# pangenome/gfasort

Hardware: AMD Instinct MI355X
Metric: SGD term-updates/sec, -p Y, 1M-node synthetic GFA (higher is better)
Workload: dtype f64

## Files before the change

gfasort_amd/csrc/host/graph.cpp:

```cpp
#include "graph.hpp"

#include <algorithm>
#include <atomic>
#include <cerrno>
#include <chrono>
#include <cstdlib>
#include <cstdio>
#include <cstring>
#include <exception>
#include <functional>
#include <stdexcept>
#include <thread>

#include <sched.h>

namespace gfasort {

namespace {
std::atomic<size_t> g_io_threads{0};

void parallel_for_impl(size_t n, const std::function<void(size_t)> &fn) {
    size_t nt = std::min(io_threads(), n);
    if (nt <= 1) { for (size_t i = 0; i < n; ++i) fn(i); return; }
    std::atomic<size_t> next{0};
// ... 79 lines not shown
        }
        add_edge(list[k].from, list[k].to);
    }
}

bool BidirectedGraph::has_edge(Handle from, Handle to) const {
    return edges.count(BiEdge{from, to}) || edges.count(BiEdge{to.flip(), from.flip()});
}

size_t BidirectedGraph::node_count() const {
    size_t n = 0;
    for (const auto &x : nodes) n += x.has_value();
    return n;
}

std::vector<size_t> BidirectedGraph::seeding_order() const {
    if (!node_order.empty()) return node_order;
    std::vector<size_t> ids;
    for (size_t id = 0; id < nodes.size(); ++id) if (nodes[id].has_value()) ids.push_back(id);
    return ids;
}

FlatGraph BidirectedGraph::flatten() const {
    FlatGraph f;
    std::vector<uint32_t> idx_of(nodes.size(), GFS_NO_NODE);
    for (size_t id : seeding_order()) {
        if (id < nodes.size() && nodes[id].has_value()) {
            if (idx_of[id] != GFS_NO_NODE) continue;
            idx_of[id] = (uint32_t)f.node_len.size();
            f.node_len.push_back((uint32_t)nodes[id]->sequence.size());
            f.node_ids.push_back(id);
        }
    }
    f.path_first_step.push_back(0);
    for (const auto &p : paths)
        f.path_first_step.push_back(f.path_first_step.back() + p.steps.size());
    f.step_node.resize(f.path_first_step.back());
    f.step_is_rev.resize(f.path_first_step.back());
    const auto chunks = step_chunks(paths, (size_t)1 << 18);
    parallel_for(chunks.size(), [&](size_t c) {
        const StepChunk &ck = chunks[c];
        const Handle *st = paths[ck.path].steps.data();
        uint32_t *sn = f.step_node.data() + f.path_first_step[ck.path];
        uint8_t *sr = f.step_is_rev.data() + f.path_first_step[ck.path];
        for (size_t k = ck.begin; k < ck.end; ++k) {
            size_t id = st[k].node_id();
            sn[k] = id < idx_of.size() ? idx_of[id] : GFS_NO_NODE;
            sr[k] = st[k].is_reverse() ? 1 : 0;
        }
    });
    return f;
}

void BidirectedGraph::apply_ordering(const std::vector<Handle> &ordering) {
    if (ordering.empty()) return;
    size_t max_old = nodes.size();
    for (Handle h : ordering) max_old = std::max(max_old, h.node_id() + 1);
    std::vector<size_t> old_to_new(max_old, 0);
    for (size_t k = 0; k < ordering.size(); ++k) old_to_new[ordering[k].node_id()] = k + 1;
    auto lookup = [&](size_t id) -> size_t { return id < old_to_new.size() ? old_to_new[id] : 0; };
    size_t max_new = 0;
    for (size_t v : old_to_new) max_new = std::max(max_new, v);
    std::vector<std::optional<BiNode>> new_nodes(max_new + 1);
    {
        const size_t BLOCK = (size_t)1 << 16;
        parallel_for((nodes.size() + BLOCK - 1) / BLOCK, [&](size_t b) {
            for (size_t id = b * BLOCK; id < std::min(nodes.size(), (b + 1) * BLOCK); ++id) {
                size_t nid = lookup(id);
                if (nid && nodes[id].has_value()) {
                    BiNode n = std::move(*nodes[id]);
                    n.id = nid;
                    n.rank = (uint64_t)(nid - 1);
                    new_nodes[nid] = std::move(n);
                }
            }
        });
    }
    nodes = std::move(new_nodes);
    std::vector<BiEdge> relabelled(edges.begin(), edges.end());
    {
        std::vector<uint8_t> keep(relabelled.size(), 0);
        const size_t BLOCK = (size_t)1 << 16;
        parallel_for((relabelled.size() + BLOCK - 1) / BLOCK, [&](size_t b) {
            for (size_t k = b * BLOCK; k < std::min(relabelled.size(), (b + 1) * BLOCK); ++k) {
                const BiEdge e = relabelled[k];
                size_t f = lookup(e.from.node_id()), t = lookup(e.to.node_id());
                if (f && t) { relabelled[k] = BiEdge{Handle::make(f, e.from.is_reverse()), Handle::make(t, e.to.is_reverse())}; keep[k] = 1; }
            }
        });
        size_t n = 0;
        for (size_t k = 0; k < relabelled.size(); ++k) if (keep[k]) relabelled[n++] = relabelled[k];
        relabelled.resize(n);
    }
    EdgeSet new_edges;
    new_edges.reserve(relabelled.size());
    for (size_t k = 0; k < relabelled.size(); ++k) {
        if (k + 16 < relabelled.size()) new_edges.prefetch(relabelled[k + 16]);
        new_edges.insert(relabelled[k]);
    }
    edges = std::move(new_edges);
    const auto chunks = step_chunks(paths, (size_t)1 << 18);
    parallel_for(chunks.size(), [&](size_t c) {
        const StepChunk &ck = chunks[c];
        Handle *st = paths[ck.path].steps.data();
        for (size_t k = ck.begin; k < ck.end; ++k) {
            size_t nid = lookup(st[k].node_id());
            if (nid) st[k] = Handle::make(nid, st[k].is_reverse());
        }
    });
}

namespace {
inline void put_uint(std::string &b, uint64_t v) {
    char tmp[24]; int n = 24;
    do { tmp[--n] = (char)('0' + v % 10); v /= 10; } while (v);
    b.append(tmp + n, (size_t)(24 - n));
}
}

namespace {
void write_blocks(std::ostream &out, size_t n, size_t block, const std::function<void(size_t, size_t, std::string &)> &fmt) {
    const size_t nblocks = (n + block - 1) / block;
    const size_t window = std::max<size_t>(io_threads() * 4, 1);
    std::vector<std::string> piece(std::min(window, std::max<size_t>(nblocks, 1)));
    for (size_t base = 0; base < nblocks; base += window) {
        const size_t cnt = std::min(window, nblocks - base);
        parallel_for(cnt, [&](size_t i) {
            piece[i].clear();
            fmt((base + i) * block, std::min(n, (base + i + 1) * block), piece[i]);
        });
        for (size_t i = 0; i < cnt; ++i) out.write(piece[i].data(), (std::streamsize)piece[i].size());
    }
}
}

void BidirectedGraph::write_gfa(std::ostream &out) const {
    const bool timing = std::getenv("GFS_TIMING") != nullptr;
    auto t_prev = std::chrono::steady_clock::now();
    auto lap = [&](const char *what) {
        if (!timing) return;
        auto t = std::chrono::steady_clock::now();
        std::fprintf(stderr, "[write_gfa] %-10s %8.2f ms\n", what, std::chrono::duration<double, std::milli>(t - t_prev).count());
        t_prev = t;
    };
    std::string b;
    b.reserve(9u << 20);
    auto flush = [&](bool force) { if (force || b.size() > (8u << 20)) { out.write(b.data(), (std::streamsize)b.size()); b.clear(); } };
    b += "H\tVN:Z:1.0\n";
    flush(true);
    write_blocks(out, nodes.size(), (size_t)1 << 16, [&](size_t lo, size_t hi, std::string &o) {
        for (size_t id = lo; id < hi; ++id)
            if (nodes[id].has_value()) {
                o += "S\t"; put_uint(o, id); o.push_back('\t'); o += nodes[id]->sequence; o.push_back('\n');
            }
    });
    lap("S");
    std::vector<BiEdge> es(edges.begin(), edges.end());
    lap("L copy");
    {
        auto less = [](const BiEdge &a, const BiEdge &c) { return a.from.v != c.from.v ? a.from.v < c.from.v : a.to.v < c.to.v; };
        size_t runs = 1;
        while (runs * 2 <= io_threads() && es.size() / (runs * 2) >= 65536) runs *= 2;
        auto bound = [&](size_t r, size_t of) { return es.size() * r / of; };
        parallel_for(runs, [&](size_t r) { std::sort(es.begin() + (std::ptrdiff_t)bound(r, runs), es.begin() + (std::ptrdiff_t)bound(r + 1, runs), less); });
        for (size_t width = 1; width < runs; width *= 2)
            parallel_for(runs / (2 * width), [&](size_t m) {
                const size_t lo = bound(2 * width * m, runs), mid = bound(2 * width * m + width, runs), hi = bound(2 * width * (m + 1), runs);
                std::inplace_merge(es.begin() + (std::ptrdiff_t)lo, es.begin() + (std::ptrdiff_t)mid, es.begin() + (std::ptrdiff_t)hi, less);
            });
    }
    lap("L sort");
    write_blocks(out, es.size(), (size_t)1 << 16, [&](size_t lo, size_t hi, std::string &o) {
        o.reserve((hi - lo) * 28);
        for (size_t k = lo; k < hi; ++k) {
            const BiEdge &e = es[k];
            o += "L\t"; put_uint(o, e.from.node_id()); o.push_back('\t'); o.push_back(e.from.orientation_char());
            o.push_back('\t'); put_uint(o, e.to.node_id()); o.push_back('\t'); o.push_back(e.to.orientation_char());
            o += "\t0M\n";
        }
    });
    lap("L");
    const auto chunks = step_chunks(paths, (size_t)1 << 17);
    const size_t window = std::max<size_t>(io_threads() * 4, 1);
    std::vector<std::string> piece(std::min(window, chunks.size()));
    size_t next_path = 0;
    auto header = [&](size_t p) { b += "P\t"; b += paths[p].name; b.push_back('\t'); };
    auto close_paths_before = [&](size_t p, bool started) {
        if (started) b += "\t*\n";
        for (; next_path < p; ++next_path) { header(next_path); b += "\t*\n"; }
    };
    bool started = false;
    for (size_t base = 0; base < chunks.size(); base += window) {
        const size_t n = std::min(window, chunks.size() - base);
        parallel_for(n, [&](size_t i) {
            const StepChunk &ck = chunks[base + i];
            const Handle *st = paths[ck.path].steps.data();
            std::string &o = piece[i];
            o.clear();
            o.reserve((ck.end - ck.begin) * 10);
            for (size_t k = ck.begin; k < ck.end; ++k) {
                if (k) o.push_back(',');
                put_uint(o, st[k].node_id()); o.push_back(st[k].orientation_char());
            }
        });
        for (size_t i = 0; i < n; ++i) {
            const StepChunk &ck = chunks[base + i];
            if (ck.begin == 0) {
                close_paths_before(ck.path, started);
                header(ck.path); next_path = ck.path + 1; started = true;
            }
            flush(true);
            out.write(piece[i].data(), (std::streamsize)piece[i].size());
        }
    }
    close_paths_before(paths.size(), started);
    flush(true);
    lap("P");
}

namespace {
struct Line { const char *b, *e; };
inline bool field(const Line &ln, int k, const char *&fb, const char *&fe) {
    const char *p = ln.b;
    for (int i = 0; i < k; ++i) {
        const char *t = (const char *)memchr(p, '\t', (size_t)(ln.e - p));
        if (!t) return false;
        p = t + 1;
    }
    const char *t = (const char *)memchr(p, '\t', (size_t)(ln.e - p));
    fb = p; fe = t ? t : ln.e;
    return true;
}
inline int count_fields(const Line &ln) {
    int n = 1;
    for (const char *p = ln.b; (p = (const char *)memchr(p, '\t', (size_t)(ln.e - p))); ++p) ++n;
    return n;
}
size_t parse_usize(const char *b, const char *e, const char *what) {
    if (b < e && *b == '+') ++b;
    if (b >= e) throw std::runtime_error(std::string("Failed to parse ") + what + ": cannot parse integer from empty string");
    uint64_t v = 0;
    for (; b < e; ++b) {
        if (*b < '0' || *b > '9') throw std::runtime_error(std::string("Failed to parse ") + what + ": invalid digit found in string");
        const uint64_t d = (uint64_t)(*b - '0');
        if (v > 1844674407370955161ull || (v == 1844674407370955161ull && d > 5))
            throw std::runtime_error(std::string("Failed to parse ") + what + ": number too large to fit in target type");
        v = v * 10 + d;
    }
    return (size_t)v;
}
}

BidirectedGraph parse_gfa(const std::string &content) {
    BidirectedGraph g;
    const bool timing = std::getenv("GFS_TIMING") != nullptr;
// ... 168 lines not shown
```

gfasort_amd/csrc/host/graph.hpp:

```cpp
#pragma once
#include <cstdint>
#include <functional>
#include <optional>
#include <ostream>
#include <string>
#include <iterator>
#include <vector>

#include "../../../include/gfasort_hip.h"

namespace gfasort {

struct Handle {
    uint64_t v = 0;
    static Handle make(size_t node_id, bool is_reverse) { return Handle{((uint64_t)node_id << 1) | (is_reverse ? 1u : 0u)}; }
    static Handle forward(size_t node_id) { return make(node_id, false); }
    static Handle reverse(size_t node_id) { return make(node_id, true); }
    static Handle from_u64(uint64_t x) { return Handle{x}; }
    size_t node_id() const { return (size_t)(v >> 1); }
    bool is_reverse() const { return (v & 1) == 1; }
    char orientation_char() const { return is_reverse() ? '-' : '+'; }
    Handle flip() const { return Handle{v ^ 1}; }
    uint64_t as_u64() const { return v; }
    bool operator==(const Handle &o) const { return v == o.v; }
// ... 34 lines not shown
        const BiEdge *operator->() const { return &s_->slots_[i_]; }
        const_iterator &operator++() { ++i_; skip(); return *this; }
        bool operator!=(const const_iterator &o) const { return i_ != o.i_; }
        bool operator==(const const_iterator &o) const { return i_ == o.i_; }
        using iterator_category = std::forward_iterator_tag;
        using value_type = BiEdge; using difference_type = std::ptrdiff_t;
        using pointer = const BiEdge *; using reference = const BiEdge &;
    private:
        void skip() { while (i_ < s_->used_.size() && !s_->used_[i_]) ++i_; }
        const EdgeSet *s_; size_t i_;
    };
    size_t size() const { return n_; }
    bool empty() const { return n_ == 0; }
    void clear() { slots_.clear(); used_.clear(); n_ = 0; }
    void reserve(size_t n) { if (n * 10 > slots_.size() * 7) rehash(n); }
    size_t count(const BiEdge &e) const {
        if (slots_.empty()) return 0;
        const size_t mask = slots_.size() - 1;
        for (size_t i = BiEdgeHash()(e) & mask;; i = (i + 1) & mask) {
            if (!used_[i]) return 0;
            if (slots_[i] == e) return 1;
        }
    }
    bool insert(const BiEdge &e) {
        if ((n_ + 1) * 10 > slots_.size() * 7) rehash(n_ + 1);
        const size_t mask = slots_.size() - 1;
        for (size_t i = BiEdgeHash()(e) & mask;; i = (i + 1) & mask) {
            if (!used_[i]) { slots_[i] = e; used_[i] = 1; ++n_; return true; }
            if (slots_[i] == e) return false;
        }
    }
    void prefetch(const BiEdge &e) const {
        if (slots_.empty()) return;
        const size_t i = BiEdgeHash()(e) & (slots_.size() - 1);
        __builtin_prefetch(&slots_[i]); __builtin_prefetch(&used_[i]);
    }
    const_iterator begin() const { return const_iterator(this, 0); }
    const_iterator end() const { return const_iterator(this, used_.size()); }
private:
    void rehash(size_t want) {
        size_t cap = 16;
        while (cap * 7 < want * 10) cap <<= 1;
        if (cap < slots_.size()) cap = slots_.size();
        std::vector<BiEdge> old_s(cap); std::vector<uint8_t> old_u(cap, 0);
        old_s.swap(slots_); old_u.swap(used_);
        n_ = 0;
        for (size_t i = 0; i < old_u.size(); ++i) if (old_u[i]) insert(old_s[i]);
    }
    std::vector<BiEdge> slots_;
    std::vector<uint8_t> used_;
    size_t n_ = 0;
};

struct FlatGraph {
    std::vector<uint32_t> node_len;
    std::vector<uint32_t> step_node;
    std::vector<uint8_t> step_is_rev;
    std::vector<uint64_t> path_first_step;
    std::vector<size_t> node_ids;
    gfs_graph_view view() const {
        gfs_graph_view v;
        v.n_nodes = node_len.size(); v.n_steps = step_node.size(); v.n_paths = path_first_step.size() - 1;
        v.node_len = node_len.data(); v.step_node = step_node.data();
        v.step_is_rev = step_is_rev.data(); v.path_first_step = path_first_step.data();
        return v;
    }
};

struct BidirectedGraph {
    std::vector<std::optional<BiNode>> nodes;
    EdgeSet edges;
    std::vector<BiPath> paths;
    std::vector<size_t> node_order;

    void add_node(size_t id, std::string sequence);
    void add_edge(Handle from, Handle to);
    void add_edges(const std::vector<BiEdge> &list);
    bool has_edge(Handle from, Handle to) const;
    size_t node_count() const;
    void apply_ordering(const std::vector<Handle> &ordering);
    void write_gfa(std::ostream &out) const;
    std::vector<size_t> seeding_order() const;
    FlatGraph flatten() const;
};

void set_io_threads(size_t n);
size_t io_threads();
void parallel_for(size_t n, const std::function<void(size_t)> &fn);

std::string read_file(const std::string &path);

BidirectedGraph parse_gfa(const std::string &content);

}
```

gfasort_amd/csrc/host/main.cpp:

```cpp
#include <chrono>
#include <cstdlib>
#include <cstring>
#include <fstream>
#include <iostream>
#include <sstream>
#include <string>
#include <thread>

#include "sgd.hpp"

using namespace gfasort;

struct Args {
    std::string input, output, pipeline = "sYgs", layout_out;
    size_t iter_max = 100, threads = 1, dimensions = 2, layout_iter = 30;
    unsigned verbose = 1;
    uint64_t streams = 0; uint32_t flags = 0;
    unsigned bundle = 0;
    bool reference_sampler = false, phased = false;
};

static void usage() {
    std::cerr <<
        "Usage: gfasort_hip -i <in.gfa> -o <out.gfa> [-p PIPELINE] [--iter-max N] [-t N] [-v N]\n"
// ... 20 lines not shown
        std::string f = argv[i];
        const char *v;
        if (f == "-i" || f == "--input") { if (!(v = need(i))) return false; a.input = v; }
        else if (f == "-o" || f == "--output") { if (!(v = need(i))) return false; a.output = v; }
        else if (f == "-p" || f == "--pipeline") { if (!(v = need(i))) return false; a.pipeline = v; }
        else if (f == "--iter-max") { if (!(v = need(i))) return false; a.iter_max = std::stoull(v); }
        else if (f == "-t" || f == "--threads") { if (!(v = need(i))) return false; a.threads = std::stoull(v); }
        else if (f == "-v" || f == "--verbose") { if (!(v = need(i))) return false; a.verbose = (unsigned)std::stoul(v); }
        else if (f == "--dimensions") { if (!(v = need(i))) return false; a.dimensions = std::stoull(v); }
        else if (f == "--layout-out") { if (!(v = need(i))) return false; a.layout_out = v; }
        else if (f == "--layout-iter") { if (!(v = need(i))) return false; a.layout_iter = std::stoull(v); }
        else if (f == "--io-threads") { if (!(v = need(i))) return false; set_io_threads(std::stoull(v)); }
        else if (f == "--streams") { if (!(v = need(i))) return false; a.streams = std::stoull(v); }
        else if (f == "--bundle") { if (!(v = need(i))) return false; a.bundle = std::string(v) == "auto" ? 0u : (unsigned)std::stoul(v); }
        else if (f == "--reference-sampler") { a.bundle = 1; a.reference_sampler = true; }
        else if (f == "--phased-sampler") { a.phased = true; }
        else if (f == "--hip-flags") { if (!(v = need(i))) return false; a.flags = (uint32_t)std::stoul(v); }
        else if (f == "-h" || f == "--help") { usage(); exit(0); }
        else { std::cerr << "error: unexpected argument '" << f << "'\n"; return false; }
    }
    if (a.phased && (a.reference_sampler || (a.bundle != 0 && a.bundle != 64))) {
        std::cerr << "error: --phased-sampler switches between the reference sampler and bundles of 64: not with --reference-sampler or --bundle "
                  << a.bundle << "\n";
        return false;
    }
    if (a.input.empty() || a.output.empty()) { std::cerr << "error: -i and -o are required\n"; return false; }
    return true;
}

static int validate_pipeline(const std::string &p) {
    for (char c : p) {
        switch (c) {
            case 'Y': case 'L': break;
            case 'g': case 's': case 'S': case 'u':
                std::cerr << "Error: pipeline step '" << c << "' is part of the reference but not of this build "
                             "(only Y = SGD and L = layout run on the HIP engine)\n";
                return 1;
            default:
                std::cerr << "Error: Unknown pipeline character '" << c
                          << "'. Valid: Y (SGD), g (groom), s (topo-sort), S (priority-topo-sort), u (unchop), L (layout)\n";
                return 1;
        }
    }
    if (p.empty()) { std::cerr << "Error: Pipeline cannot be empty\n"; return 1; }
    return 0;
}

int main(int argc, char **argv) {
    Args args;
    if (!parse_args(argc, argv, args)) { usage(); return 2; }
    if (validate_pipeline(args.pipeline)) return 1;
    auto t_start = std::chrono::steady_clock::now();
    auto since = [&](std::chrono::steady_clock::time_point t0) { return std::chrono::duration<double>(std::chrono::steady_clock::now() - t0).count(); };
    double t_read = 0, t_parse = 0, t_steps = 0, t_write = 0;
    std::thread warm([] { (void)gfs_warmup(0); });
    struct Joiner { std::thread &t; ~Joiner() { if (t.joinable()) t.join(); } } joiner{warm};
    if (args.verbose >= 1) std::cerr << "[gfasort] reading " << args.input << "\n";
    std::string content;
    try { content = read_file(args.input); }
    catch (const std::exception &e) { std::cerr << "Error reading file: " << e.what() << "\n"; return 1; }
    t_read = since(t_start);
    auto t_p0 = std::chrono::steady_clock::now();
    BidirectedGraph graph;
    try { graph = parse_gfa(content); }
    catch (const std::exception &e) { std::cerr << "Error parsing GFA: " << e.what() << "\n"; return 1; }
    t_parse = since(t_p0);
    if (args.verbose >= 1)
        std::cerr << "[gfasort] loaded " << graph.node_count() << " nodes, " << graph.edges.size() << " edges, "
                  << graph.paths.size() << " paths\n";
    if (args.verbose >= 2) std::cerr << "[gfasort] pipeline: " << args.pipeline << "\n";

    YgsParams ygs = YgsParams::from_graph(graph, (uint8_t)args.verbose, args.threads);
    PathSGDParams sgd_params = ygs.path_sgd;
    sgd_params.iter_max = args.iter_max;
    LayoutSGDParams layout_params = LayoutSGDParams::from_graph(graph, args.dimensions, args.threads);
    layout_params.iter_max = args.layout_iter;
    layout_params.progress = args.verbose >= 2;
    HipOptions opt; opt.cfg.n_streams = args.streams; opt.cfg.flags = args.flags | GFS_F_BUNDLE(args.bundle);

    bool have_layout = false;
    Layout layout;
    auto t_s0 = std::chrono::steady_clock::now();
    try {
        size_t step = 0;
        for (char c : args.pipeline) {
            ++step;
            if (args.verbose >= 1)
                std::cerr << "[gfasort] [" << step << "/" << args.pipeline.size() << "] "
                          << (c == 'Y' ? std::string("SGD") : std::to_string(args.dimensions) + "D layout") << "\n";
            gfs_stats st{};
            if (c == 'Y') {
                HipOptions opt_y = opt;
                if (args.phased) opt_y.cfg.flags |= GFS_F_PHASED;
                sgd_sort_only(graph, sgd_params, (uint8_t)args.verbose, opt_y, &st);
                if (args.phased && args.verbose >= 2) {
                    uint64_t kb = 0, ke = sgd_params.iter_max + 1;
                    if (st.bundle == 64) { gfs_sgd_params cp = sgd_params.to_c(); gfs_phase_window(&cp, &kb, &ke); }
                    std::cerr << "[gfasort_hip] phased sampler: reference streams in iterations [" << kb << ", " << ke << ") of 0.."
                              << sgd_params.iter_max << "\n";
                }
            } else {
                layout = path_linear_sgd_layout(graph, layout_params, opt, &st);
                have_layout = true;
                if (args.verbose >= 1) {
                    double stress = calculate_layout_stress(graph, layout, 10000);
                    char buf[64]; snprintf(buf, sizeof buf, "%.6f", stress);
                    std::cerr << "[gfasort] layout stress: " << buf << "\n";
                }
            }
            if (args.verbose >= 1 && st.iterations)
                std::cerr << "[gfasort_hip] " << st.term_updates << " term updates in " << st.iterations << " iterations on "
                          << st.n_streams << " streams (bundle " << st.bundle << "); kernels " << st.kernel_ms << " ms ("
                          << (st.kernel_ms > 0 ? (double)st.term_updates / st.kernel_ms / 1e6 : 0.0) << " G updates/s), call "
                          << st.total_ms << " ms\n";
        }
    } catch (const std::exception &e) {
        std::cerr << "Error: " << e.what() << "\n";
        return 1;
    }
    t_steps = since(t_s0);
    if (warm.joinable()) warm.join();
    auto t_w0 = std::chrono::steady_clock::now();
    if (have_layout) {
        if (!args.layout_out.empty()) {
            if (args.verbose >= 1) std::cerr << "[gfasort] writing layout to " << args.layout_out << "\n";
            std::ofstream f(args.layout_out, std::ios::binary);
            if (!f) { std::cerr << "Error creating layout file: " << std::strerror(errno) << "\n"; return 1; }
            layout.write_tsv(f);
        } else if (args.verbose >= 1) {
            std::cerr << "[gfasort] warning: layout computed but --layout-out not specified\n";
        }
    }
    if (args.verbose >= 1) std::cerr << "[gfasort] writing " << args.output << "\n";
    {
        std::ofstream f(args.output, std::ios::binary);
        if (!f) { std::cerr << "Error writing output file: " << std::strerror(errno) << "\n"; return 1; }
        graph.write_gfa(f);
    }
    t_write = since(t_w0);
    if (args.verbose >= 1) {
        double s = std::chrono::duration<double>(std::chrono::steady_clock::now() - t_start).count();
        std::cerr << "[gfasort] done (" << s << " s wall: read " << t_read << ", parse " << t_parse << ", pipeline "
                  << t_steps << ", write " << t_write << ")\n";
    }
    std::cerr.flush(); std::cout.flush();
    std::_Exit(0);
}
```

gfasort_amd/csrc/host/selftest.cpp:

```cpp
#include <cmath>
#include <fstream>
#include <iostream>
#include <sstream>

#include "sgd.hpp"

using namespace gfasort;
#define REQUIRE(c) do { if (!(c)) { std::cerr << "FAIL " << __FILE__ << ":" << __LINE__ << " " #c "\n"; return 1; } } while (0)

static std::string slurp(const std::string &p) { std::ifstream f(p, std::ios::binary); std::ostringstream s; s << f.rdbuf(); return s.str(); }

int main(int argc, char **argv) {
    std::string data = argc > 1 ? argv[1] : "tests/data";
    {
        Handle h1 = Handle::forward(42);
        REQUIRE(h1.node_id() == 42 && !h1.is_reverse() && h1.orientation_char() == '+');
        Handle h2 = Handle::reverse(42);
        REQUIRE(h2.node_id() == 42 && h2.is_reverse() && h2.orientation_char() == '-');
        REQUIRE(h2.as_u64() == 85 && Handle::from_u64(85) == h2);
        Handle h3 = Handle::forward(10).flip();
        REQUIRE(h3.node_id() == 10 && h3.is_reverse() && h3.flip() == Handle::forward(10));
        REQUIRE(Handle::reverse(7).to_string() == "7-");
        std::cout << "ok handle\n";
    }
// ... 23 lines not shown
        REQUIRE((g.node_order == std::vector<size_t>{1, 2, 3}));
        g.apply_ordering({});
        REQUIRE(g.node_count() == 3);
        std::cout << "ok graph\n";
    }
    {
        Layout l(2, 10);
        REQUIRE(l.coords.size() == 40);
        Layout m(2, 5);
        m.set(2, 0, 0, 100); m.set(2, 0, 1, 200); m.set(2, 1, 0, 150); m.set(2, 1, 1, 250);
        REQUIRE(m.get(2, 0, 0) == 100 && m.get(2, 0, 1) == 200 && m.get(2, 1, 0) == 150 && m.get(2, 1, 1) == 250);
        Layout d(2, 2); d.set(1, 0, 0, 3); d.set(1, 0, 1, 4);
        REQUIRE(std::fabs(d.distance(0, 0, 1, 0) - 5.0) < 1e-10);
        Layout v = Layout::from_vectors({{1, 2, 3, 4}, {10, 20, 30, 40}});
        REQUIRE(v.num_nodes == 2 && v.dimensions == 2 && v.get(0, 0, 0) == 1 && v.get(0, 0, 1) == 10 && v.get(0, 1, 0) == 2
                && v.get(0, 1, 1) == 20 && v.get(1, 0, 0) == 3 && v.get(1, 0, 1) == 30);
        Layout t(2, 1); t.set(0, 0, 0, 1.5); t.set(0, 0, 1, 10.0); t.set(0, 1, 0, 0.1 + 0.2); t.set(0, 1, 1, 1e21);
        std::ostringstream out; t.write_tsv(out);
        REQUIRE(out.str() == "idx\tx+\ty+\tx-\ty-\n0\t1.5\t10\t0.30000000000000004\t1000000000000000000000\n");
        REQUIRE(rust_display_f64(1e-7) == "0.0000001" && rust_display_f64(-0.5) == "-0.5");
        std::cout << "ok layout\n";
    }
    {
        YgsParams y;
        REQUIRE(y.path_sgd.iter_max == 100 && y.path_sgd.theta == 0.99 && y.path_sgd.eps == 0.01);
        PathSGDParams d;
        REQUIRE(d.min_term_updates == 100 && d.eta_max == 100.0 && d.space == 100 && d.space_max == 100 && d.seed == 9399220);
        LayoutSGDParams lp;
        REQUIRE(lp.dimensions == 2 && lp.iter_max == 30 && lp.space_max == 1000);
        BidirectedGraph g;
        g.add_node(1, "AAAA"); g.add_node(2, "CCCC"); g.add_node(3, "GGGG");
        BiPath p; p.name = "t"; p.add_step(Handle::forward(1)); p.add_step(Handle::forward(2)); p.add_step(Handle::forward(3));
        g.paths.push_back(p);
        YgsParams f = YgsParams::from_graph(g, 0, 1);
        REQUIRE(f.path_sgd.min_term_updates == 3 && f.path_sgd.eta_max == 9.0 && f.path_sgd.space == 12);
        std::cout << "ok params\n";
    }
    struct Row { const char *name; size_t nodes, steps, paths; uint64_t ymin; double yeta; uint64_t yspace, lmin; uint64_t lspace; };
    Row table[] = { {"simple.gfa", 15, 10, 1, 10, 100.0, 50, 100, 10}, {"lil.gfa", 15, 30, 3, 30, 100.0, 50, 300, 10},
                    {"DRB1-3123.gfa", 4955, 35059, 12, 35059, 9610000.0, 15931, 350590, 3100} };
    for (const Row &r : table) {
        std::string txt = slurp(data + "/" + r.name);
        REQUIRE(!txt.empty());
        BidirectedGraph g = parse_gfa(txt);
        FlatGraph f = g.flatten();
        REQUIRE(g.node_count() == r.nodes && f.step_node.size() == r.steps && g.paths.size() == r.paths);
        YgsParams y = YgsParams::from_graph(g, 0, 1);
        REQUIRE(y.path_sgd.min_term_updates == r.ymin && y.path_sgd.eta_max == r.yeta && y.path_sgd.space == r.yspace);
        LayoutSGDParams lp = LayoutSGDParams::from_graph(g, 2, 1);
        REQUIRE(lp.min_term_updates == r.lmin && lp.eta_max == r.yeta && lp.space == r.lspace);
        std::ostringstream out; g.write_gfa(out);
        BidirectedGraph g2 = parse_gfa(out.str());
        REQUIRE(g2.node_count() == g.node_count() && g2.edges.size() == g.edges.size() && g2.paths.size() == g.paths.size());
        gfs_sgd_params cp = y.path_sgd.to_c();
        std::vector<double> etas(cp.iter_max + 1);
        REQUIRE(gfs_sgd_schedule(&cp, etas.data()) == 0 && etas[0] == 1.0 / (1.0 / r.yeta));
        std::cout << "ok fixture " << r.name << "\n";
    }
    {
        BidirectedGraph g;
        REQUIRE(path_linear_sgd(g, PathSGDParams()).empty());
        REQUIRE(path_sgd_sort(g, PathSGDParams()).empty());
        Layout l = path_linear_sgd_layout(g, LayoutSGDParams());
        REQUIRE(l.num_nodes == 0 && l.dimensions == 2);
        std::cout << "ok empty\n";
    }
    {
        std::string small = "S\t1\tA\nS\t2\tC\nS\t3\tG\nP\tp\t1+,, 2- ,3+ ,\t*\nP\tempty\t\t*\nP\tq\t3x,+2+\t*\n";
        for (size_t nt : {1, 3}) {
            set_io_threads(nt);
            BidirectedGraph g = parse_gfa(small);
            REQUIRE(g.paths.size() == 3 && g.paths[1].steps.empty());
            REQUIRE((g.paths[0].steps == std::vector<Handle>{Handle::forward(1), Handle::reverse(2), Handle::forward(3)}));
            REQUIRE((g.paths[2].steps == std::vector<Handle>{Handle::reverse(3), Handle::forward(2)}));
            std::ostringstream out; g.write_gfa(out);
            REQUIRE(out.str().find("P\tp\t1+,2-,3+\t*\nP\tempty\t\t*\nP\tq\t3-,2+\t*\n") != std::string::npos);
            std::string big = "S\t1\tA\nP\tlong\t";
            std::vector<Handle> want;
            for (size_t k = 0; k < 700000; ++k) {
                size_t id = 1 + (k * 2654435761u) % 999983;
                bool rev = (k % 7) == 3;
                big += std::to_string(id); big += rev ? '-' : '+'; big += ',';
                if (k % 1000 == 999) big += " ,";
                want.push_back(Handle::make(id, rev));
            }
            big += "\t*\n";
            BidirectedGraph gb = parse_gfa(big);
            REQUIRE(gb.paths.size() == 1 && gb.paths[0].steps == want);
            FlatGraph f = gb.flatten();
            REQUIRE(f.step_node.size() == want.size() && f.step_is_rev[3] == 1 && f.step_node[0] == 0 && f.step_node[1] == GFS_NO_NODE);
            std::ostringstream ob; gb.write_gfa(ob);
            BidirectedGraph gb2 = parse_gfa(ob.str());
            REQUIRE(gb2.paths[0].steps == want);
            std::string bad = big; bad.replace(bad.size() - 20, 1, "x");
            bool threw = false;
            try { (void)parse_gfa(bad); } catch (const std::exception &e) {
                threw = std::string(e.what()) == "Failed to parse path node ID: invalid digit found in string";
            }
            REQUIRE(threw);
            threw = false;
            try { (void)parse_gfa("P\tp\t99999999999999999999+\t*\n"); } catch (const std::exception &e) {
                threw = std::string(e.what()) == "Failed to parse path node ID: number too large to fit in target type";
            }
            REQUIRE(threw);
            REQUIRE(parse_gfa("P\tp\t18446744073709551615+\t*\n").paths[0].steps.size() == 1);
        }
// ... 24 lines not shown
```

gfasort_amd/csrc/host/sgd.cpp:

```cpp
#include "sgd.hpp"

#include <algorithm>
#include <charconv>
#include <chrono>
#include <cstdio>
#include <cstdlib>
#include <cmath>
#include <cstring>
#include <iostream>
#include <ostream>
#include <stdexcept>

namespace gfasort {

gfs_sgd_params PathSGDParams::to_c() const {
    gfs_sgd_params c;
    std::memset(&c, 0, sizeof c);
    c.iter_max = iter_max; c.iter_with_max_learning_rate = iter_with_max_learning_rate;
    c.min_term_updates = min_term_updates; c.delta = delta; c.eps = eps; c.eta_max = eta_max; c.theta = theta;
    c.space = space; c.space_max = space_max; c.space_quantization_step = space_quantization_step;
    c.cooling_start = cooling_start; c.nthreads = nthreads; c.progress = progress ? 1 : 0; c.seed = seed;
    return c;
}

gfs_layout_params LayoutSGDParams::to_c() const {
    PathSGDParams s;
    s.iter_max = iter_max; s.iter_with_max_learning_rate = iter_with_max_learning_rate;
    s.min_term_updates = min_term_updates; s.delta = delta; s.eps = eps; s.eta_max = eta_max; s.theta = theta;
    s.space = space; s.space_max = space_max; s.space_quantization_step = space_quantization_step;
    s.cooling_start = cooling_start; s.nthreads = nthreads; s.progress = progress; s.seed = seed;
    gfs_layout_params c;
    c.dimensions = dimensions; c.sgd = s.to_c();
    return c;
}

static void path_stats(const BidirectedGraph &g, uint64_t &sum_steps, size_t &max_steps, size_t &max_len) {
    sum_steps = 0; max_steps = 0; max_len = 0;
    for (const auto &p : g.paths) {
        size_t pos = 0;
        for (Handle h : p.steps) {
            size_t id = h.node_id();
            if (id < g.nodes.size() && g.nodes[id].has_value()) pos += g.nodes[id]->sequence.size();
        }
        sum_steps += p.steps.size();
        max_steps = std::max(max_steps, p.steps.size());
        max_len = std::max(max_len, pos);
    }
}

LayoutSGDParams LayoutSGDParams::from_graph(const BidirectedGraph &g, size_t dimensions, size_t nthreads) {
    uint64_t sum; size_t mx, ml;
    path_stats(g, sum, mx, ml);
    LayoutSGDParams p;
    p.dimensions = dimensions; p.iter_max = 30; p.min_term_updates = 10 * sum;
    p.eta_max = (double)(mx * mx); p.space = mx; p.space_max = 1000; p.space_quantization_step = 100;
    p.nthreads = nthreads;
    return p;
}

YgsParams::YgsParams() {
    path_sgd.iter_max = 100; path_sgd.min_term_updates = 0; path_sgd.eta_max = 0.0; path_sgd.space = 0;
    path_sgd.space_max = 100; path_sgd.space_quantization_step = 100;
}

YgsParams YgsParams::from_graph(const BidirectedGraph &g, uint8_t verbose, size_t nthreads) {
    YgsParams y;
    y.verbose = verbose;
    y.path_sgd.nthreads = nthreads;
    y.path_sgd.progress = verbose >= 2;
    uint64_t sum; size_t mx, ml;
    path_stats(g, sum, mx, ml);
    y.path_sgd.min_term_updates = sum;
    y.path_sgd.eta_max = (double)(mx * mx);
    y.path_sgd.space = ml;
    if (verbose >= 2) {
        std::cerr << "[ygs_sort] Calculated parameters:\n  sum_path_step_count: " << sum
                  << "\n  max_path_step_count: " << mx << "\n  max_path_length: " << ml
                  << "\n  min_term_updates: " << y.path_sgd.min_term_updates
                  << "\n  eta_max: " << rust_display_f64(y.path_sgd.eta_max) << "\n  space: " << y.path_sgd.space << "\n";
    }
    return y;
}

Layout Layout::from_vectors(const std::vector<std::vector<double>> &v) {
    if (v.empty()) throw std::runtime_error("Must have at least 1 dimension");
    size_t entries = v[0].size();
    if (entries % 2) throw std::runtime_error("Must have even number of entries (2 per node)");
    for (const auto &d : v) if (d.size() != entries) throw std::runtime_error("All dimension vectors must have same length");
    Layout l(v.size(), entries / 2);
    for (size_t node = 0; node < l.num_nodes; ++node)
        for (size_t end = 0; end < 2; ++end)
            for (size_t dim = 0; dim < l.dimensions; ++dim) l.coords[l.index(node, end, dim)] = v[dim][node * 2 + end];
    return l;
}

double Layout::distance(size_t na, size_t ea, size_t nb, size_t eb) const {
    double s = 0.0;
    for (size_t d = 0; d < dimensions; ++d) { double delta = get(na, ea, d) - get(nb, eb, d); s += delta * delta; }
    return std::sqrt(s);
}

std::string rust_display_f64(double v) {
    if (v != v) return "NaN";
    if (std::isinf(v)) return v > 0 ? "inf" : "-inf";
    char buf[512];
    auto r = std::to_chars(buf, buf + sizeof buf, v, std::chars_format::fixed);
    return std::string(buf, r.ptr);
}

static const char *dim_name(size_t d) {
    switch (d) { case 0: return "x"; case 1: return "y"; case 2: return "z"; case 3: return "w"; default: return "d"; }
}

void Layout::write_tsv(std::ostream &out) const {
    out << "idx";
    for (size_t d = 0; d < dimensions; ++d) out << "\t" << dim_name(d) << "+";
    for (size_t d = 0; d < dimensions; ++d) out << "\t" << dim_name(d) << "-";
    out << "\n";
    const size_t BLOCK = 1 << 14, nblocks = (num_nodes + BLOCK - 1) / BLOCK;
    const size_t window = std::max<size_t>(io_threads() * 4, 1);
    std::vector<std::string> piece(std::min(window, std::max<size_t>(nblocks, 1)));
    for (size_t base = 0; base < nblocks; base += window) {
        const size_t n = std::min(window, nblocks - base);
        parallel_for(n, [&](size_t i) {
// ... 15 lines not shown
                    }
                o.push_back('\n');
            }
        });
        for (size_t i = 0; i < n; ++i) out.write(piece[i].data(), (std::streamsize)piece[i].size());
    }
}

static void check(int rc) {
    if (rc < 0) throw std::runtime_error(std::string("gfasort_hip: ") + gfs_last_error());
}

static std::vector<double> path_linear_sgd_vec(const BidirectedGraph &g, const FlatGraph &f, const PathSGDParams &p,
                                               const HipOptions &opt, gfs_stats *stats) {
    std::vector<double> x;
    if (g.node_count() == 0) return x;
    gfs_graph_view v = f.view();
    gfs_sgd_params cp = p.to_c();
    x.resize(f.node_len.size());
    gfs_stats st;
    int rc = gfs_path_linear_sgd(&v, &cp, &opt.cfg, nullptr, nullptr, 1, x.data(), &st);
    check(rc);
    if (stats) *stats = st;
    if (rc == GFS_NOTHING_TO_DO) {
        std::cerr << "[path_sgd] No paths with multiple steps found\n";
        x.clear();
    }
    return x;
}

std::unordered_map<size_t, double> path_linear_sgd(const BidirectedGraph &g, const PathSGDParams &p,
                                                   const HipOptions &opt, gfs_stats *stats) {
    std::unordered_map<size_t, double> positions;
    FlatGraph f = g.flatten();
    std::vector<double> x = path_linear_sgd_vec(g, f, p, opt, stats);
    positions.reserve(x.size());
    for (size_t i = 0; i < x.size(); ++i) positions.emplace(i, x[i]);
    return positions;
}

namespace {
struct Lap {
    bool on = std::getenv("GFS_TIMING") != nullptr;
    std::chrono::steady_clock::time_point t = std::chrono::steady_clock::now();
    void operator()(const char *what) {
        if (!on) return;
        auto n = std::chrono::steady_clock::now();
        std::fprintf(stderr, "[sgd_sort] %-14s %8.2f ms\n", what, std::chrono::duration<double, std::milli>(n - t).count());
        t = n;
    }
};
}

std::vector<Handle> path_sgd_sort(const BidirectedGraph &g, const PathSGDParams &p, const HipOptions &opt,
                                  gfs_stats *stats) {
    std::vector<Handle> out;
    if (g.node_count() == 0) return out;
    Lap lap;
    FlatGraph f = g.flatten();
    lap("flatten");
    gfs_graph_view v = f.view();
    gfs_sgd_params cp = p.to_c();
    std::vector<double> x(f.node_len.size());
    std::vector<uint64_t> order(x.size());
    gfs_stats st;
    int rc = gfs_path_sgd_sort(&v, &cp, &opt.cfg, nullptr, nullptr, 1, x.data(), order.data(), &st);
    lap("gfs_path_sgd_sort");
    check(rc);
    if (stats) *stats = st;
    if (rc == GFS_NOTHING_TO_DO) {
        std::cerr << "[path_sgd] No paths with multiple steps found\n";
        return out;
    }
    out.reserve(order.size());
    for (uint64_t idx : order) out.push_back(Handle::forward(f.node_ids[idx]));
    lap("handles");
    return out;
}

void sgd_sort_only(BidirectedGraph &g, const PathSGDParams &p, uint8_t verbose, const HipOptions &opt, gfs_stats *stats) {
    if (verbose >= 2) std::cerr << "[path_sgd] Starting path-guided SGD\n";
    auto ordering = path_sgd_sort(g, p, opt, stats);
    Lap lap;
    g.apply_ordering(ordering);
    lap("apply_ordering");
    if (verbose >= 2) std::cerr << "[path_sgd] Complete\n";
}

static uint64_t splitmix64(uint64_t &s) {
    uint64_t z = (s += 0x9E3779B97F4A7C15ull);
    z = (z ^ (z >> 30)) * 0xBF58476D1CE4E5B9ull;
    z = (z ^ (z >> 27)) * 0x94D049BB133111EBull;
    return z ^ (z >> 31);
}

std::vector<double> default_layout_init(const FlatGraph &f, size_t D, uint64_t seed) {
    const size_t N = f.node_len.size(), n = N * 2 * D;
    std::vector<double> c(n, 0.0);
    gfs_graph_view v = f.view();
    gfs_init_layout(&v, D, seed, c.data());
    return c;
}

Layout path_linear_sgd_layout(const BidirectedGraph &g, const LayoutSGDParams &p, const HipOptions &opt, gfs_stats *stats) {
    size_t N = g.node_count();
    if (N == 0) return Layout(p.dimensions, 0);
    FlatGraph f = g.flatten();
    gfs_graph_view v = f.view();
    gfs_layout_params cp = p.to_c();
    std::vector<double> coords = default_layout_init(f, p.dimensions, p.seed);
    gfs_stats st;
    int rc = gfs_path_linear_sgd_layout(&v, &cp, &opt.cfg, nullptr, nullptr, coords.data(), &st);
    check(rc);
    if (stats) *stats = st;
    if (rc == GFS_NOTHING_TO_DO) {
        std::cerr << "[path_sgd_layout] No paths with multiple steps found\n";
        return Layout(p.dimensions, N);
    }
    Layout l(p.dimensions, N);
    l.coords = std::move(coords);
    return l;
}

namespace {
struct Xo {
    uint64_t s[4];
    explicit Xo(uint64_t seed) { uint64_t sm = seed; for (auto &v : s) v = splitmix64(sm); }
    uint64_t next() {
        uint64_t r = s[0] + s[3], t = s[1] << 17;
        s[2] ^= s[0]; s[3] ^= s[1]; s[1] ^= s[2]; s[0] ^= s[3]; s[2] ^= t;
        s[3] = (s[3] << 45) | (s[3] >> 19);
        return r;
    }
    uint64_t uniform(uint64_t n) {
        if (n <= 0xFFFFFFFFull) {
            uint32_t range = (uint32_t)n, thresh = (uint32_t)(0u - range) % range;
            for (;;) { uint64_t m = (uint64_t)(uint32_t)(next() >> 32) * range; if ((uint32_t)m >= thresh) return m >> 32; }
        }
        uint64_t thresh = (0ull - n) % n;
        for (;;) { unsigned __int128 m = (unsigned __int128)next() * n; if ((uint64_t)m >= thresh) return (uint64_t)(m >> 64); }
    }
};
}

double calculate_layout_stress(const BidirectedGraph &g, const Layout &layout, size_t sample_count) {
    FlatGraph f = g.flatten();
    const size_t S = f.step_node.size();
    if (S < 2) return 0.0;
    std::vector<uint64_t> pos(S); std::vector<uint32_t> pth(S);
    for (size_t p = 0; p + 1 < f.path_first_step.size(); ++p) {
        uint64_t position = 0;
        for (uint64_t s = f.path_first_step[p]; s < f.path_first_step[p + 1]; ++s) {
            pos[s] = position; pth[s] = (uint32_t)p;
            if (f.step_node[s] != GFS_NO_NODE) position += f.node_len[f.step_node[s]];
        }
    }
    Xo rng(12345);
    double sum = 0.0; uint64_t count = 0;
    for (size_t k = 0; k < sample_count; ++k) {
        uint64_t a = rng.uniform(S);
        uint64_t p = pth[a], first = f.path_first_step[p], cnt = f.path_first_step[p + 1] - first;
        if (cnt < 2) continue;
        uint64_t ra = a - first, rb = rng.uniform(cnt);
        if (ra == rb) continue;
        uint64_t sa = first + ra, sb = first + rb;
        double path_dist = std::fabs((double)pos[sa] - (double)pos[sb]);
        if (path_dist == 0.0) continue;
        uint32_t ia = f.step_node[sa], ib = f.step_node[sb];
        if (ia == GFS_NO_NODE || ib == GFS_NO_NODE) continue;
        double err = layout.distance(ia, 0, ib, 0) - path_dist;
        sum += (err * err) / (path_dist * path_dist);
        ++count;
    }
    return count ? std::sqrt(sum / (double)count) : 0.0;
}

}
```

gfasort_amd/csrc/host/sgd.hpp:

```cpp
#pragma once
#include <cstdint>
#include <iosfwd>
#include <string>
#include <unordered_map>
#include <vector>

#include "graph.hpp"

namespace gfasort {

struct PathSGDParams {
    uint64_t iter_max = 100;
    uint64_t iter_with_max_learning_rate = 0;
    uint64_t min_term_updates = 100;
    double delta = 0.0;
    double eps = 0.01;
    double eta_max = 100.0;
    double theta = 0.99;
    uint64_t space = 100;
    uint64_t space_max = 100;
    uint64_t space_quantization_step = 100;
    double cooling_start = 0.5;
    size_t nthreads = 1;
    bool progress = false;
    uint64_t seed = 9399220;
    gfs_sgd_params to_c() const;
};

struct LayoutSGDParams {
    size_t dimensions = 2;
    uint64_t iter_max = 30;
    uint64_t iter_with_max_learning_rate = 0;
    uint64_t min_term_updates = 100;
    double delta = 0.0;
    double eps = 0.01;
    double eta_max = 100.0;
    double theta = 0.99;
    uint64_t space = 100;
    uint64_t space_max = 1000;
    uint64_t space_quantization_step = 100;
    double cooling_start = 0.5;
    size_t nthreads = 1;
    bool progress = false;
    uint64_t seed = 9399220;
    static LayoutSGDParams from_graph(const BidirectedGraph &g, size_t dimensions, size_t nthreads);
    gfs_layout_params to_c() const;
};

struct YgsParams {
    PathSGDParams path_sgd;
    uint8_t verbose = 0;
    YgsParams();
    static YgsParams from_graph(const BidirectedGraph &g, uint8_t verbose, size_t nthreads);
};

struct Layout {
    size_t dimensions = 0;
    size_t num_nodes = 0;
    std::vector<double> coords;
    Layout() = default;
    Layout(size_t dims, size_t n) : dimensions(dims), num_nodes(n), coords(n * 2 * dims, 0.0) {}
    static Layout from_vectors(const std::vector<std::vector<double>> &coord_vecs);
    size_t index(size_t node, size_t end, size_t dim) const { return node * 2 * dimensions + end * dimensions + dim; }
    double get(size_t node, size_t end, size_t dim) const { return coords[index(node, end, dim)]; }
    void set(size_t node, size_t end, size_t dim, double v) { coords[index(node, end, dim)] = v; }
    double distance(size_t na, size_t ea, size_t nb, size_t eb) const;
    void write_tsv(std::ostream &out) const;
};

std::string rust_display_f64(double v);

struct HipOptions {
    gfs_launch_config cfg{};
};

std::unordered_map<size_t, double> path_linear_sgd(const BidirectedGraph &g, const PathSGDParams &p,
                                                   const HipOptions &opt = {}, gfs_stats *stats = nullptr);
std::vector<Handle> path_sgd_sort(const BidirectedGraph &g, const PathSGDParams &p, const HipOptions &opt = {},
                                  gfs_stats *stats = nullptr);
void sgd_sort_only(BidirectedGraph &g, const PathSGDParams &p, uint8_t verbose, const HipOptions &opt = {},
                   gfs_stats *stats = nullptr);
Layout path_linear_sgd_layout(const BidirectedGraph &g, const LayoutSGDParams &p, const HipOptions &opt = {},
                              gfs_stats *stats = nullptr);
std::vector<double> default_layout_init(const FlatGraph &f, size_t dims, uint64_t seed);
double calculate_layout_stress(const BidirectedGraph &g, const Layout &layout, size_t sample_count);

}
```

Baseline: 104.3 billion.

## Reuse flattened graph, compute path stats from it, and write ordered GFA directly

Flattens the graph once in main, derives path statistics from the flat arrays in parallel, and passes the flat graph into SGD sort, layout and stress instead of re-flattening each time. For the last Y step it skips apply_ordering and instead remaps node IDs while writing the GFA. The goal is to remove redundant host-side flatten, stats and reordering work around the GPU kernel. It adds a second output code path whose result must match apply_ordering followed by write_gfa.

```diff
diff --git a/gfasort_amd/csrc/host/graph.cpp b/gfasort_amd/csrc/host/graph.cpp
--- a/gfasort_amd/csrc/host/graph.cpp
+++ b/gfasort_amd/csrc/host/graph.cpp
@@ -155,6 +155,31 @@
     return f;
 }
 
+PathStats FlatGraph::path_stats() const {
+    PathStats st;
+    const size_t P = path_first_step.size() - 1, CHUNK = (size_t)1 << 18;
+    struct Part { size_t path; uint64_t begin, end, bp; };
+    std::vector<Part> parts;
+    for (size_t p = 0; p < P; ++p)
+        for (uint64_t b = path_first_step[p]; b < path_first_step[p + 1]; b += CHUNK)
+            parts.push_back(Part{p, b, std::min<uint64_t>(path_first_step[p + 1], b + CHUNK), 0});
+    parallel_for(parts.size(), [&](size_t i) {
+        uint64_t bp = 0;
+        for (uint64_t s = parts[i].begin; s < parts[i].end; ++s)
+            if (step_node[s] != GFS_NO_NODE) bp += node_len[step_node[s]];
+        parts[i].bp = bp;
+    });
+    std::vector<uint64_t> len(P, 0);
+    for (const Part &pt : parts) len[pt.path] += pt.bp;
+    for (size_t p = 0; p < P; ++p) {
+        const size_t steps = (size_t)(path_first_step[p + 1] - path_first_step[p]);
+        st.sum_steps += steps;
+        st.max_steps = std::max(st.max_steps, steps);
+        st.max_len = std::max(st.max_len, (size_t)len[p]);
+    }
+    return st;
+}
+
 void BidirectedGraph::apply_ordering(const std::vector<Handle> &ordering) {
     if (ordering.empty()) return;
     size_t max_old = nodes.size();
@@ -237,7 +262,18 @@
 }
 }
 
-void BidirectedGraph::write_gfa(std::ostream &out) const {
+void BidirectedGraph::write_gfa(std::ostream &out) const { write_gfa_impl(out, nullptr); }
+
+void BidirectedGraph::write_gfa_ordered(std::ostream &out, const std::vector<Handle> &ordering) const {
+    if (ordering.empty()) { write_gfa_impl(out, nullptr); return; }
+    size_t max_old = nodes.size();
+    for (Handle h : ordering) max_old = std::max(max_old, h.node_id() + 1);
+    std::vector<size_t> old_to_new(max_old, 0);
+    for (size_t k = 0; k < ordering.size(); ++k) old_to_new[ordering[k].node_id()] = k + 1;
+    write_gfa_impl(out, &old_to_new);
+}
+
+void BidirectedGraph::write_gfa_impl(std::ostream &out, const std::vector<size_t> *old_to_new) const {
     const bool timing = std::getenv("GFS_TIMING") != nullptr;
     auto t_prev = std::chrono::steady_clock::now();
     auto lap = [&](const char *what) {
@@ -251,14 +287,39 @@
     auto flush = [&](bool force) { if (force || b.size() > (8u << 20)) { out.write(b.data(), (std::streamsize)b.size()); b.clear(); } };
     b += "H\tVN:Z:1.0\n";
     flush(true);
-    write_blocks(out, nodes.size(), (size_t)1 << 16, [&](size_t lo, size_t hi, std::string &o) {
-        for (size_t id = lo; id < hi; ++id)
-            if (nodes[id].has_value()) {
-                o += "S\t"; put_uint(o, id); o.push_back('\t'); o += nodes[id]->sequence; o.push_back('\n');
-            }
+    auto lookup = [&](size_t id) -> size_t { return id < old_to_new->size() ? (*old_to_new)[id] : 0; };
+    constexpr size_t NONE = ~(size_t)0;
+    std::vector<size_t> new_to_old;
+    if (old_to_new) {
+        size_t max_new = 0;
+        for (size_t v : *old_to_new) max_new = std::max(max_new, v);
+        new_to_old.assign(max_new + 1, NONE);
+        for (size_t id = 0; id < nodes.size(); ++id) {
+            const size_t nid = lookup(id);
+            if (nid && nodes[id].has_value()) new_to_old[nid] = id;
+        }
+    }
+    const size_t n_ids = old_to_new ? new_to_old.size() : nodes.size();
+    write_blocks(out, n_ids, (size_t)1 << 14, [&](size_t lo, size_t hi, std::string &o) {
+        o.reserve((hi - lo) * 24);
+        for (size_t id = lo; id < hi; ++id) {
+            const size_t src = old_to_new ? new_to_old[id] : id;
+            if (src != NONE && nodes[src].has_value()) {
+                o += "S\t"; put_uint(o, id); o.push_back('\t'); o += nodes[src]->sequence; o.push_back('\n');
+            }
+        }
     });
     lap("S");
     std::vector<BiEdge> es(edges.begin(), edges.end());
+    if (old_to_new) {
+        size_t n = 0;
+        for (size_t k = 0; k < es.size(); ++k) {
+            const BiEdge e = es[k];
+            const size_t f = lookup(e.from.node_id()), t = lookup(e.to.node_id());
+            if (f && t) es[n++] = BiEdge{Handle::make(f, e.from.is_reverse()), Handle::make(t, e.to.is_reverse())};
+        }
+        es.resize(n);
+    }
     lap("L copy");
     {
         auto less = [](const BiEdge &a, const BiEdge &c) { return a.from.v != c.from.v ? a.from.v < c.from.v : a.to.v < c.to.v; };
@@ -303,7 +364,9 @@
             o.reserve((ck.end - ck.begin) * 10);
             for (size_t k = ck.begin; k < ck.end; ++k) {
                 if (k) o.push_back(',');
-                put_uint(o, st[k].node_id()); o.push_back(st[k].orientation_char());
+                size_t id = st[k].node_id();
+                if (old_to_new) { const size_t nid = lookup(id); if (nid) id = nid; }
+                put_uint(o, id); o.push_back(st[k].orientation_char());
             }
         });
         for (size_t i = 0; i < n; ++i) {
diff --git a/gfasort_amd/csrc/host/graph.hpp b/gfasort_amd/csrc/host/graph.hpp
--- a/gfasort_amd/csrc/host/graph.hpp
+++ b/gfasort_amd/csrc/host/graph.hpp
@@ -110,6 +110,8 @@
     size_t n_ = 0;
 };
 
+struct PathStats { uint64_t sum_steps = 0; size_t max_steps = 0, max_len = 0; };
+
 struct FlatGraph {
     std::vector<uint32_t> node_len;
     std::vector<uint32_t> step_node;
@@ -123,6 +125,7 @@
         v.step_is_rev = step_is_rev.data(); v.path_first_step = path_first_step.data();
         return v;
     }
+    PathStats path_stats() const;
 };
 
 struct BidirectedGraph {
@@ -138,8 +141,11 @@
     size_t node_count() const;
     void apply_ordering(const std::vector<Handle> &ordering);
     void write_gfa(std::ostream &out) const;
+    void write_gfa_ordered(std::ostream &out, const std::vector<Handle> &ordering) const;
     std::vector<size_t> seeding_order() const;
     FlatGraph flatten() const;
+private:
+    void write_gfa_impl(std::ostream &out, const std::vector<size_t> *old_to_new) const;
 };
 
 void set_io_threads(size_t n);
diff --git a/gfasort_amd/csrc/host/main.cpp b/gfasort_amd/csrc/host/main.cpp
--- a/gfasort_amd/csrc/host/main.cpp
+++ b/gfasort_amd/csrc/host/main.cpp
@@ -96,7 +96,7 @@
     if (validate_pipeline(args.pipeline)) return 1;
     auto t_start = std::chrono::steady_clock::now();
     auto since = [&](std::chrono::steady_clock::time_point t0) { return std::chrono::duration<double>(std::chrono::steady_clock::now() - t0).count(); };
-    double t_read = 0, t_parse = 0, t_steps = 0, t_write = 0;
+    double t_read = 0, t_parse = 0, t_prep = 0, t_steps = 0, t_write = 0;
     std::thread warm([] { (void)gfs_warmup(0); });
     struct Joiner { std::thread &t; ~Joiner() { if (t.joinable()) t.join(); } } joiner{warm};
     if (args.verbose >= 1) std::cerr << "[gfasort] reading " << args.input << "\n";
@@ -114,16 +114,24 @@
                   << graph.paths.size() << " paths\n";
     if (args.verbose >= 2) std::cerr << "[gfasort] pipeline: " << args.pipeline << "\n";
 
-    YgsParams ygs = YgsParams::from_graph(graph, (uint8_t)args.verbose, args.threads);
+    auto t_f0 = std::chrono::steady_clock::now();
+    const bool wants_layout = args.pipeline.find('L') != std::string::npos;
+    FlatGraph flat = graph.flatten();
+    const PathStats path_stats = flat.path_stats();
+    YgsParams ygs = YgsParams::from_stats(path_stats, (uint8_t)args.verbose, args.threads);
     PathSGDParams sgd_params = ygs.path_sgd;
     sgd_params.iter_max = args.iter_max;
-    LayoutSGDParams layout_params = LayoutSGDParams::from_graph(graph, args.dimensions, args.threads);
+    LayoutSGDParams layout_params;
+    if (wants_layout) layout_params = LayoutSGDParams::from_stats(path_stats, args.dimensions, args.threads);
     layout_params.iter_max = args.layout_iter;
     layout_params.progress = args.verbose >= 2;
+    t_prep = since(t_f0);
     HipOptions opt; opt.cfg.n_streams = args.streams; opt.cfg.flags = args.flags | GFS_F_BUNDLE(args.bundle);
 
     bool have_layout = false;
     Layout layout;
+    std::vector<Handle> final_order;
+    bool flat_is_current = true;
     auto t_s0 = std::chrono::steady_clock::now();
     try {
         size_t step = 0;
@@ -136,7 +144,11 @@
             if (c == 'Y') {
                 HipOptions opt_y = opt;
                 if (args.phased) opt_y.cfg.flags |= GFS_F_PHASED;
-                sgd_sort_only(graph, sgd_params, (uint8_t)args.verbose, opt_y, &st);
+                const bool last = step == args.pipeline.size();
+                if (!flat_is_current) { flat = graph.flatten(); flat_is_current = true; }
+                auto order = sgd_sort_only(graph, flat, !last, sgd_params, (uint8_t)args.verbose, opt_y, &st);
+                if (last) final_order = std::move(order);
+                else flat_is_current = order.empty();
                 if (args.phased && args.verbose >= 2) {
                     uint64_t kb = 0, ke = sgd_params.iter_max + 1;
                     if (st.bundle == 64) { gfs_sgd_params cp = sgd_params.to_c(); gfs_phase_window(&cp, &kb, &ke); }
@@ -144,10 +156,11 @@
                               << sgd_params.iter_max << "\n";
                 }
             } else {
-                layout = path_linear_sgd_layout(graph, layout_params, opt, &st);
+                if (!flat_is_current) { flat = graph.flatten(); flat_is_current = true; }
+                layout = path_linear_sgd_layout(graph, flat, layout_params, opt, &st);
                 have_layout = true;
                 if (args.verbose >= 1) {
-                    double stress = calculate_layout_stress(graph, layout, 10000);
+                    double stress = calculate_layout_stress(flat, layout, 10000);
                     char buf[64]; snprintf(buf, sizeof buf, "%.6f", stress);
                     std::cerr << "[gfasort] layout stress: " << buf << "\n";
                 }
@@ -179,12 +192,12 @@
     {
         std::ofstream f(args.output, std::ios::binary);
         if (!f) { std::cerr << "Error writing output file: " << std::strerror(errno) << "\n"; return 1; }
-        graph.write_gfa(f);
+        graph.write_gfa_ordered(f, final_order);
     }
     t_write = since(t_w0);
     if (args.verbose >= 1) {
         double s = std::chrono::duration<double>(std::chrono::steady_clock::now() - t_start).count();
-        std::cerr << "[gfasort] done (" << s << " s wall: read " << t_read << ", parse " << t_parse << ", pipeline "
+        std::cerr << "[gfasort] done (" << s << " s wall: read " << t_read << ", parse " << t_parse << ", flatten " << t_prep << ", pipeline "
                   << t_steps << ", write " << t_write << ")\n";
     }
     std::cerr.flush(); std::cout.flush();
diff --git a/gfasort_amd/csrc/host/selftest.cpp b/gfasort_amd/csrc/host/selftest.cpp
--- a/gfasort_amd/csrc/host/selftest.cpp
+++ b/gfasort_amd/csrc/host/selftest.cpp
@@ -99,6 +99,29 @@
         std::ostringstream out; g.write_gfa(out);
         BidirectedGraph g2 = parse_gfa(out.str());
         REQUIRE(g2.node_count() == g.node_count() && g2.edges.size() == g.edges.size() && g2.paths.size() == g.paths.size());
+        YgsParams ys = YgsParams::from_stats(f.path_stats(), 0, 1);
+        LayoutSGDParams ls = LayoutSGDParams::from_stats(f.path_stats(), 2, 1);
+        REQUIRE(ys.path_sgd.min_term_updates == r.ymin && ys.path_sgd.eta_max == r.yeta && ys.path_sgd.space == r.yspace);
+        REQUIRE(ls.min_term_updates == r.lmin && ls.eta_max == r.yeta && ls.space == r.lspace);
+        for (int partial = 0; partial < 2; ++partial)
+            for (size_t nt : {1, 3}) {
+                set_io_threads(nt);
+                std::vector<Handle> ord;
+                const size_t n = f.node_ids.size();
+                for (size_t k = 0; k < n; ++k)
+                    if (!partial || k % 5) ord.push_back(Handle::forward(f.node_ids[(k * 7 + 3) % n]));
+                if (partial) { ord.push_back(ord[1]); ord.push_back(Handle::forward(g.nodes.size() + 3)); }
+                std::ostringstream direct; g.write_gfa_ordered(direct, ord);
+                BidirectedGraph h = parse_gfa(txt);
+                h.apply_ordering(ord);
+                std::ostringstream rebuilt; h.write_gfa(rebuilt);
+                REQUIRE(direct.str() == rebuilt.str() && direct.str() != out.str());
+            }
+        set_io_threads(0);
+        {
+            std::ostringstream same; g.write_gfa_ordered(same, {});
+            REQUIRE(same.str() == out.str());
+        }
         gfs_sgd_params cp = y.path_sgd.to_c();
         std::vector<double> etas(cp.iter_max + 1);
         REQUIRE(gfs_sgd_schedule(&cp, etas.data()) == 0 && etas[0] == 1.0 / (1.0 / r.yeta));
diff --git a/gfasort_amd/csrc/host/sgd.cpp b/gfasort_amd/csrc/host/sgd.cpp
--- a/gfasort_amd/csrc/host/sgd.cpp
+++ b/gfasort_amd/csrc/host/sgd.cpp
@@ -49,8 +49,13 @@
 }
 
 LayoutSGDParams LayoutSGDParams::from_graph(const BidirectedGraph &g, size_t dimensions, size_t nthreads) {
-    uint64_t sum; size_t mx, ml;
-    path_stats(g, sum, mx, ml);
+    PathStats s;
+    path_stats(g, s.sum_steps, s.max_steps, s.max_len);
+    return from_stats(s, dimensions, nthreads);
+}
+
+LayoutSGDParams LayoutSGDParams::from_stats(const PathStats &s, size_t dimensions, size_t nthreads) {
+    const uint64_t sum = s.sum_steps; const size_t mx = s.max_steps;
     LayoutSGDParams p;
     p.dimensions = dimensions; p.iter_max = 30; p.min_term_updates = 10 * sum;
     p.eta_max = (double)(mx * mx); p.space = mx; p.space_max = 1000; p.space_quantization_step = 100;
@@ -64,12 +69,17 @@
 }
 
 YgsParams YgsParams::from_graph(const BidirectedGraph &g, uint8_t verbose, size_t nthreads) {
+    PathStats s;
+    path_stats(g, s.sum_steps, s.max_steps, s.max_len);
+    return from_stats(s, verbose, nthreads);
+}
+
+YgsParams YgsParams::from_stats(const PathStats &s, uint8_t verbose, size_t nthreads) {
     YgsParams y;
     y.verbose = verbose;
     y.path_sgd.nthreads = nthreads;
     y.path_sgd.progress = verbose >= 2;
-    uint64_t sum; size_t mx, ml;
-    path_stats(g, sum, mx, ml);
+    const uint64_t sum = s.sum_steps; const size_t mx = s.max_steps, ml = s.max_len;
     y.path_sgd.min_term_updates = sum;
     y.path_sgd.eta_max = (double)(mx * mx);
     y.path_sgd.space = ml;
@@ -191,13 +201,21 @@
 };
 }
 
+static std::vector<Handle> path_sgd_sort_flat(const FlatGraph &f, const PathSGDParams &p, const HipOptions &opt, gfs_stats *stats);
+
 std::vector<Handle> path_sgd_sort(const BidirectedGraph &g, const PathSGDParams &p, const HipOptions &opt,
                                   gfs_stats *stats) {
-    std::vector<Handle> out;
-    if (g.node_count() == 0) return out;
+    if (g.node_count() == 0) return {};
     Lap lap;
     FlatGraph f = g.flatten();
     lap("flatten");
+    return path_sgd_sort_flat(f, p, opt, stats);
+}
+
+static std::vector<Handle> path_sgd_sort_flat(const FlatGraph &f, const PathSGDParams &p, const HipOptions &opt, gfs_stats *stats) {
+    std::vector<Handle> out;
+    if (f.node_len.empty()) return out;
+    Lap lap;
     gfs_graph_view v = f.view();
     gfs_sgd_params cp = p.to_c();
     std::vector<double> x(f.node_len.size());
@@ -226,6 +244,19 @@
     if (verbose >= 2) std::cerr << "[path_sgd] Complete\n";
 }
 
+std::vector<Handle> sgd_sort_only(BidirectedGraph &g, const FlatGraph &f, bool apply, const PathSGDParams &p, uint8_t verbose,
+                                  const HipOptions &opt, gfs_stats *stats) {
+    if (verbose >= 2) std::cerr << "[path_sgd] Starting path-guided SGD\n";
+    auto ordering = path_sgd_sort_flat(f, p, opt, stats);
+    if (apply) {
+        Lap lap;
+        g.apply_ordering(ordering);
+        lap("apply_ordering");
+    }
+    if (verbose >= 2) std::cerr << "[path_sgd] Complete\n";
+    return ordering;
+}
+
 static uint64_t splitmix64(uint64_t &s) {
     uint64_t z = (s += 0x9E3779B97F4A7C15ull);
     z = (z ^ (z >> 30)) * 0xBF58476D1CE4E5B9ull;
@@ -242,9 +273,14 @@
 }
 
 Layout path_linear_sgd_layout(const BidirectedGraph &g, const LayoutSGDParams &p, const HipOptions &opt, gfs_stats *stats) {
+    if (g.node_count() == 0) return Layout(p.dimensions, 0);
+    return path_linear_sgd_layout(g, g.flatten(), p, opt, stats);
+}
+
+Layout path_linear_sgd_layout(const BidirectedGraph &g, const FlatGraph &f, const LayoutSGDParams &p, const HipOptions &opt,
+                              gfs_stats *stats) {
     size_t N = g.node_count();
     if (N == 0) return Layout(p.dimensions, 0);
-    FlatGraph f = g.flatten();
     gfs_graph_view v = f.view();
     gfs_layout_params cp = p.to_c();
     std::vector<double> coords = default_layout_init(f, p.dimensions, p.seed);
@@ -283,7 +319,10 @@
 }
 
 double calculate_layout_stress(const BidirectedGraph &g, const Layout &layout, size_t sample_count) {
-    FlatGraph f = g.flatten();
+    return calculate_layout_stress(g.flatten(), layout, sample_count);
+}
+
+double calculate_layout_stress(const FlatGraph &f, const Layout &layout, size_t sample_count) {
     const size_t S = f.step_node.size();
     if (S < 2) return 0.0;
     std::vector<uint64_t> pos(S); std::vector<uint32_t> pth(S);
diff --git a/gfasort_amd/csrc/host/sgd.hpp b/gfasort_amd/csrc/host/sgd.hpp
--- a/gfasort_amd/csrc/host/sgd.hpp
+++ b/gfasort_amd/csrc/host/sgd.hpp
@@ -44,6 +44,7 @@
     bool progress = false;
     uint64_t seed = 9399220;
     static LayoutSGDParams from_graph(const BidirectedGraph &g, size_t dimensions, size_t nthreads);
+    static LayoutSGDParams from_stats(const PathStats &s, size_t dimensions, size_t nthreads);
     gfs_layout_params to_c() const;
 };
 
@@ -52,6 +53,7 @@
     uint8_t verbose = 0;
     YgsParams();
     static YgsParams from_graph(const BidirectedGraph &g, uint8_t verbose, size_t nthreads);
+    static YgsParams from_stats(const PathStats &s, uint8_t verbose, size_t nthreads);
 };
 
 struct Layout {
@@ -80,9 +82,14 @@
                                   gfs_stats *stats = nullptr);
 void sgd_sort_only(BidirectedGraph &g, const PathSGDParams &p, uint8_t verbose, const HipOptions &opt = {},
                    gfs_stats *stats = nullptr);
+std::vector<Handle> sgd_sort_only(BidirectedGraph &g, const FlatGraph &f, bool apply, const PathSGDParams &p, uint8_t verbose,
+                                  const HipOptions &opt = {}, gfs_stats *stats = nullptr);
 Layout path_linear_sgd_layout(const BidirectedGraph &g, const LayoutSGDParams &p, const HipOptions &opt = {},
+                              gfs_stats *stats = nullptr);
+Layout path_linear_sgd_layout(const BidirectedGraph &g, const FlatGraph &f, const LayoutSGDParams &p, const HipOptions &opt = {},
                               gfs_stats *stats = nullptr);
 std::vector<double> default_layout_init(const FlatGraph &f, size_t dims, uint64_t seed);
 double calculate_layout_stress(const BidirectedGraph &g, const Layout &layout, size_t sample_count);
+double calculate_layout_stress(const FlatGraph &f, const Layout &layout, size_t sample_count);
 
 }
```

Result: no change. 104.2 billion (-0.2%).
